# WU-CVGL/CasualHDRSplat

Measured on AMD Instinct MI355X. Metric: train-step images/sec (fwd+bwd raster) @ 1M Gaussians 1080p, higher is better.
Workload: dtype f32; 1 GPU; c3: 1000000 Gaussians, 1920x1080, SH degree 3, HDR radiance + CRF tone-map, 1 pose(s)/view, 1 view(s)/step (one per GPU); num_rendered_R=6777809, R_prime=3025699, pixel_pair_evals_E=559372855, seed=0, binning=sync-free fixed capacity 1.25*R, launch=eager (one enqueue per kernel)

## Files before the change

casualhdrsplat_amd/csrc/api.hip:

```cpp
#include <stdarg.h>
#include <stdio.h>
#include <stdlib.h>
#include <string.h>
#include <time.h>
#include <unistd.h>
#include <atomic>

#include "hs_cloud.h"

namespace hs {

static thread_local char g_err[512] = "";

#ifdef HS_TESTING
int fault_injection() {
    static const int mode = [] {
        const char* e = getenv("HS_FAULT_INJECT");
        return (e && !strcmp(e, "sort_ticket")) ? 1 : (e && !strcmp(e, "stalled_chain")) ? 2 : (e && !strcmp(e, "late_block")) ? 3 : 0;
    }();
    return mode;
}
#endif

static std::atomic<int> g_sort_tickets{0};
// ... 89 lines not shown
    l.offsets = carve(I * 4);
    l.cov3D = carve((int64_t)d.P * 6 * 4);
    l.clamped = carve(I);
    l.scan_spine = carve(((I + 255) / 256 + 1) * 4);
    l.binfo = carve(I * 8);
    sz->geom_bytes = o;
    o = 0;
    l.keys_sorted = carve(2 * align_up(d.capacity * 4, 256));
    l.point_list = l.keys_sorted + align_up(d.capacity * 4, 256);
    l.pairs_tmp = carve(d.capacity * 8);
    l.ranges = carve(vtiles * 8);
    l.sort_tmp = carve(sort_tmp_bytes(I));
    l.depth_ws = carve(depth_ws_words(I) * 4);
    l.depth_pairs = carve(2 * I * 8);
    l.inst_sorted = carve(I * 4);
    l.offs_sorted = carve(I * 4);
    l.pair_sort_tmp = carve(emit_scan_words(I) * 4 + sort_tmp_bytes(d.capacity));
    l.pair_flags = carve(d.capacity);
    l.pair_act = carve(d.capacity);
    l.tile_matrix = carve(count_matrix_words(I, vtiles, d.capacity) * 4);
    l.hier_ws = carve(hier_ws_words(I, gx, gy, d.n_poses, d.capacity) * 4);
    sz->binning_bytes = o;
    o = 0;
    l.final_T = carve(HW * d.n_poses * 4);
    l.n_contrib = carve(HW * d.n_poses * 4);
    l.pose_hdr = carve(HW * 3 * 4 * (d.n_poses + (npf > 1 ? F : 0)));
    l.tile_work = carve(vtiles * 4);
    l.tile_order = carve(vtiles * 4);
    sz->image_bytes = o;
    o = 0;
    l.pair_grads = carve(d.capacity * kPairFloats * 4);
    l.crf_partials = carve(crf_partial_floats(d.crf_K, HW, d.n_poses) * 4);
    l.inst_grads = carve(I * kInstFloats * 4);
    l.pose_partials = carve(pose_partial_floats(d.P, d.n_poses) * 4);
    sz->bwd_bytes = o;
    if (L) *L = l;
    return HS_OK;
}

static int debug_sync(int flags, hipStream_t s, const char* stage) {
    if (!(flags & HS_FLAG_DEBUG)) return HS_OK;
    const hipError_t e = hipStreamSynchronize(s);
    if (e != hipSuccess) {
        set_error("debug: stage `%s` failed: %s", stage, hipGetErrorString(e));
        return HS_EHIP;
    }
    return HS_OK;
}

static int check_common(const hs_dims& d, const float* means3D, const float* shs, const float* colors,
                        const float* scales, const float* rots, const float* cov, const float* view,
                        const float* proj, const float* campos, const float* bg, const char* who) {
    if (!means3D || !view || !proj || !campos || !bg) { set_error("%s: null required pointer", who); return HS_EINVAL; }
    if ((shs == nullptr) == (colors == nullptr)) { set_error("%s: provide exactly one of shs / colors_precomp", who); return HS_EINVAL; }
    const bool sr = scales && rots;
    if (sr == (cov != nullptr) || ((scales == nullptr) != (rots == nullptr))) {
        set_error("%s: provide exactly one of (scales, rotations) / cov3D_precomp", who);
        return HS_EINVAL;
    }
    if (shs) {
        if (d.M > 32) {
            set_error("%s: M=%d SH coefficients per channel; at most 32 are supported", who, d.M);
            return HS_EINVAL;
        }
        if (d.sh_degree < 0 || d.sh_degree > 3 || (d.sh_degree + 1) * (d.sh_degree + 1) > d.M) {
            set_error("%s: sh_degree %d needs %d coefficients, M=%d", who, d.sh_degree, (d.sh_degree + 1) * (d.sh_degree + 1), d.M);
// ... 160 lines not shown
        return HS_EINVAL;
    }
    const int ndens = (a->densify_grad_accum != nullptr) + (a->densify_denom != nullptr) + (a->densify_max_radii != nullptr);
    if (ndens != 0 && ndens != 3) {
        set_error("hs_backward: densification statistics need grad_accum, denom and max_radii together");
        return HS_EINVAL;
    }
    if (a->g_begin != 0 || a->g_end != 0) {
        if (a->g_begin < 0 || a->g_end < a->g_begin || a->g_end > a->dims.P || (a->g_begin & 127) ||
            (a->stages & ~HS_BWD_PROJECT)) {
            set_error("hs_backward: [g_begin, g_end) = [%d, %d) needs 0 <= g_begin <= g_end <= P, g_begin a multiple of 128, "
                      "and stages == HS_BWD_PROJECT", a->g_begin, a->g_end);
            return HS_EINVAL;
        }
    }
    if (a->dims.P == 0) return HS_OK;
    const bool crf_in_tail = HS_TUNE_CRF_IN_RENDER_TAIL && (a->stages & HS_BWD_RENDER) && (a->stages & HS_BWD_CRF) &&
                             !(a->flags & HS_FLAG_DEBUG) && a->crf_K <= 1024;
    if (a->stages & HS_BWD_RENDER) {
        rc = launch_render_bwd(*a, L, s, nullptr, nullptr, crf_in_tail);
        if (rc) return rc;
        if ((rc = debug_sync(a->flags, s, "render backward"))) return rc;
    }
    CrfReduce crf_reduce{nullptr, 0, 0, 0, nullptr, nullptr, 0};
    const bool sums_follow = (a->stages & (HS_BWD_PREPROCESS | HS_BWD_SEGSUM)) != 0 && !(a->flags & HS_FLAG_DEBUG);
    if (a->stages & HS_BWD_CRF) {
        rc = launch_crf_bwd(*a, L, s, sums_follow ? &crf_reduce : nullptr, crf_in_tail);
        if (rc) return rc;
        if ((rc = debug_sync(a->flags, s, "CRF gradient"))) return rc;
    }
    if (a->stages & (HS_BWD_PREPROCESS | HS_BWD_SEGSUM | HS_BWD_PROJECT)) {
        const bool whole = (a->stages & HS_BWD_PREPROCESS) != 0;
        rc = launch_preprocess_bwd(*a, L, s, whole || (a->stages & HS_BWD_SEGSUM), whole || (a->stages & HS_BWD_PROJECT),
                                   crf_reduce.nblocks ? &crf_reduce : nullptr);
        if (rc) return rc;
        if ((rc = debug_sync(a->flags, s, "preprocess backward"))) return rc;
    }
    return HS_OK;
}

int hs_depth_sort(int mode) {
    if (mode >= 0) hs::g_depth_sort.store(mode ? 1 : 0, std::memory_order_relaxed);
    const int v = hs::g_depth_sort.load(std::memory_order_relaxed);
    return v >= 0 ? v : (HS_TUNE_DEPTH_MSD_DEFAULT ? 1 : 0);
}

int hs_sort_tickets(int enable) {
    if (enable >= 0) hs::g_sort_tickets.store(enable ? 1 : 0, std::memory_order_relaxed);
    return hs::g_sort_tickets.load(std::memory_order_relaxed);
}

int hs_mark_visible(int32_t P, const float* means3D, const float* viewmatrix, uint8_t* visible, void* hip_stream) {
    if (P < 0 || (P > 0 && (!means3D || !viewmatrix || !visible))) { set_error("hs_mark_visible: bad argument"); return HS_EINVAL; }
    if (P == 0) return HS_OK;
    return launch_mark_visible(P, means3D, viewmatrix, visible, (hipStream_t)hip_stream);
}

int hs_sh_backward_views(int32_t P, int32_t M, int32_t sh_degree, int32_t V, const float* means3D, const float* camposes,
                         const float* dL_dview_colors, float* dL_dshs, void* hip_stream) {
    if (P < 0 || V < 1 || sh_degree < 0 || sh_degree > 3 || M < (sh_degree + 1) * (sh_degree + 1) || M > 16 ||
        (P > 0 && (!means3D || !camposes || !dL_dview_colors || !dL_dshs))) {
        set_error("hs_sh_backward_views: bad argument");
        return HS_EINVAL;
    }
    if (P == 0) return HS_OK;
    return launch_sh_backward_views(P, M, sh_degree, V, means3D, camposes, dL_dview_colors, dL_dshs, (hipStream_t)hip_stream);
}
// ... 130 lines not shown
```

casualhdrsplat_amd/csrc/hs_common.h:

```cpp
#pragma once
#include <hip/hip_runtime.h>
#include <stdint.h>

#include "../../include/hdrsplat.h"

#if defined(__HIP_DEVICE_COMPILE__) && !defined(__gfx950__)
#error "libhdrsplat is written for gfx950 (MI355X) only: build with --offload-arch=gfx950"
#endif

namespace hs {

void set_error(const char* fmt, ...);

#define HS_HIP_CHECK(expr)                                                                         \
    do {                                                                                           \
        hipError_t e_ = (expr);                                                                    \
        if (e_ != hipSuccess) {                                                                    \
            ::hs::set_error("%s failed: %s (%s:%d)", #expr, hipGetErrorString(e_), __FILE__, __LINE__); \
            return HS_EHIP;                                                                        \
        }                                                                                          \
    } while (0)
#define HS_LAUNCH_CHECK() HS_HIP_CHECK(hipGetLastError())

#ifndef HS_TUNE_CRF_IN_RENDER_TAIL
// ... 18 lines not shown
#endif
constexpr int kDepthSortItems = HS_TUNE_DEPTH_ITEMS, kDepthSortLook = 8;
constexpr int kPairSortItems = 16, kPairSortLook = 8;
constexpr int kU64SortItems = 16;
constexpr int kDepthTile = kDepthSortItems * kDepthBins, kPairTile = kPairSortItems * kSortBlock, kU64Tile = kU64SortItems * kSortBlock;
static_assert(kPairTile == kU64Tile && kDepthTile >= kPairTile, "the scratch of every sort is sized for the smallest tile");
constexpr int kSortTileMin = kPairTile;

static inline int64_t align_up(int64_t v, int64_t a) { return (v + a - 1) / a * a; }
static inline int ceil_div(int64_t a, int64_t b) { return (int)((a + b - 1) / b); }
constexpr int kMaxPoses = 21845;
static inline int frames_of(const hs_dims& d) { return d.n_frames > 1 ? d.n_frames : 1; }

static inline int tile_bits(uint32_t n) {
    int b = 0;
    while (n) { ++b; n >>= 1; }
    return b;
}

int launch_preprocess_fwd(const hs_fwd_args& a, const hs_layout& L, hipStream_t s, uint32_t frame_tag);
int launch_scan(const hs_fwd_args& a, const hs_layout& L, hipStream_t s);
int launch_cov3d(const hs_fwd_args& a, const hs_layout& L, hipStream_t s);
struct SortChoice;
int launch_binning(const hs_fwd_args& a, const hs_layout& L, const SortChoice& sort, hipStream_t s, uint32_t frame_tag);
int launch_empty_frame(hs_counters* clear, uint2* ranges, int64_t ntiles, uint32_t* counters_host, const hs_counters* counters,
                       hipStream_t s);
int launch_render_fwd(const hs_fwd_args& a, const hs_layout& L, hipStream_t s, unsigned long long* stats = nullptr);
int launch_render_bwd(const hs_bwd_args& a, const hs_layout& L, hipStream_t s, unsigned long long* stats = nullptr,
                      unsigned long long* timeline = nullptr, bool crf_in_tail = false);
int render_stats_count();
struct CrfReduce;
int launch_crf_bwd(const hs_bwd_args& a, const hs_layout& L, hipStream_t s, CrfReduce* defer, bool in_render_tail = false);
int launch_preprocess_bwd(const hs_bwd_args& a, const hs_layout& L, hipStream_t s, bool segsum, bool project,
                          const CrfReduce* crf_reduce);
int launch_mark_visible(int P, const float* means3D, const float* view, uint8_t* vis, hipStream_t s);
int launch_spline_poses(int J, int T, int kind, const float* delta, const float* base, const float* times, float* w2c,
                        float* jac, int* seg, hipStream_t s);
int launch_sh_backward_views(int P, int M, int deg, int V, const float* means3D, const float* camposes,
                             const float* view_colors, float* d_shs, hipStream_t s);
int64_t loss_pair_count(int planes, int H, int W);
int launch_loss_fwd(const hs_loss_args& a, hipStream_t s);
int launch_loss_bwd(const hs_loss_args& a, hipStream_t s);
int launch_activate_fwd(const hs_activate_args& a, hipStream_t s);
int launch_activate_bwd(const hs_activate_args& a, hipStream_t s);

constexpr int kGhistCopies = 16;
constexpr int kGhistWords = kGhistCopies * 8 * 256;
constexpr int kTicketWords = 128, kDepthBitsAt = 32, kDepthBitsCopies = 16, kDepthBitsWords = 4 * kDepthBitsCopies;
static_assert(kDepthBitsAt >= 8 && kDepthBitsAt % 2 == 0 && kDepthBitsAt + kDepthBitsWords <= kTicketWords, "depth bits live in the ticket row");
__host__ __device__ inline int64_t sweep_pass_words(int64_t nblk, int bins = 256) { return nblk * bins; }
static inline int64_t sort_scratch_words(int64_t n, int passes, int tile, int bins = 256) {
    return n > 0 ? kGhistWords + kTicketWords + (int64_t)passes * sweep_pass_words((n + tile - 1) / tile, bins) : 0;
}
static inline int64_t depth_scratch_words(int64_t I) { return sort_scratch_words(I, 4, kDepthTile, kDepthBins); }
int64_t sort_tmp_bytes(int64_t n);
constexpr int kMsdBits = 12, kMsdBuckets = 1 << kMsdBits;
#ifndef HS_TUNE_MSD_RANGE
#define HS_TUNE_MSD_RANGE 2048
#endif
constexpr int kMsdRange = HS_TUNE_MSD_RANGE, kMsdCap = 4096;
#ifndef HS_TUNE_MSD_SMALL_RANGE
#define HS_TUNE_MSD_SMALL_RANGE 512
#endif
static inline int depth_msd_range(int64_t I) { return I <= (1 << 18) ? HS_TUNE_MSD_SMALL_RANGE : kMsdRange; }
static inline bool depth_msd_fits(int64_t I) { return I > 0 && I < (2 << 20); }
static inline int depth_msd_tile(int64_t I) { return I <= (1 << 18) ? 1024 : 4096; }
static inline int64_t depth_msd_rows(int64_t I) { return (I + depth_msd_tile(I) - 1) / depth_msd_tile(I); }
// ... 124 lines not shown
}
__device__ __forceinline__ uint32_t wave_or_hi(uint32_t v) {
    v |= dpp_u32<0xB1>(v);
    v |= dpp_u32<0x4E>(v);
    v |= dpp_u32<0x141>(v);
    v |= dpp_u32<0x140>(v);
    v |= dpp_u32<0x142, 0xA>(v);
    v |= dpp_u32<0x143, 0xC>(v);
    return v;
}
__device__ __forceinline__ void depth_bits_accumulate2(uint32_t o_in, uint32_t nz_in, unsigned long long* bits, uint32_t tag,
                                                       uint32_t* s_two ) {
    const uint32_t o = wave_or_hi(o_in), nz = wave_or_hi(nz_in);
    if ((threadIdx.x & 63) == 63) { if (o) atomicOr(&s_two[0], o); if (nz) atomicOr(&s_two[1], nz); }
    __syncthreads();
    if (threadIdx.x < 2 && s_two[threadIdx.x])
        tagged_or(bits + 2 * (blockIdx.x % kDepthBitsCopies) + threadIdx.x, tag, s_two[threadIdx.x]);
}
__device__ __forceinline__ void depth_bits_accumulate(uint32_t key, bool visible, unsigned long long* bits, uint32_t tag,
                                                      uint32_t* s_two ) {
    depth_bits_accumulate2(visible ? key : 0u, visible ? ~key : 0u, bits, tag, s_two);
}
__device__ __forceinline__ float radiance_dact(int act, float col, bool was_clamped) {
    if (act == 1) return col;
    if (act == 2) return -expm1f(-col);
    return was_clamped ? 0.f : 1.f;
}

struct SegsumArgs {
    int64_t I;
    const uint32_t* inst_sorted; const uint32_t* offs_sorted;
    const float4* pair_grads; const uint8_t* pair_flags; float4* inst_grads; const hs_counters* counters;
    const int* radii_inst; const uint8_t* clamped; float* view_colors; const float4* rec; int act;
};
__device__ __forceinline__ void pair_segsum_body(const SegsumArgs& a, int64_t t) {
    const int64_t i = t >> 2;
    const int q = (int)(t & 3);
    const bool valid = i < a.I && !a.counters->overflow;
    const uint32_t beg = valid ? (i == 0 ? 0u : a.offs_sorted[i - 1]) : 0u;
    const uint32_t end = valid ? a.offs_sorted[i] : 0u;
    float r[10] = {0.f, 0.f, 0.f, 0.f, 0.f, 0.f, 0.f, 0.f, 0.f, 0.f};
    for (uint32_t s = beg + q; s < end; s += 8) {
        const bool two = s + 4 < end;
        const bool f0 = a.pair_flags[s] != 0;
        const bool f1 = two && a.pair_flags[s + 4] != 0;
        float4 a0 = make_float4(0.f, 0.f, 0.f, 0.f), a1 = a0, b0 = a0, b1 = a0;
        float2 a2 = make_float2(0.f, 0.f), b2 = a2;
        if (f0) {
            a0 = a.pair_grads[kPairF4 * (int64_t)s + 0];
            a1 = a.pair_grads[kPairF4 * (int64_t)s + 1];
            a2 = reinterpret_cast<const float2*>(a.pair_grads + kPairF4 * (int64_t)s + 2)[0];
        }
        if (f1) {
            b0 = a.pair_grads[kPairF4 * (int64_t)(s + 4) + 0];
            b1 = a.pair_grads[kPairF4 * (int64_t)(s + 4) + 1];
            b2 = reinterpret_cast<const float2*>(a.pair_grads + kPairF4 * (int64_t)(s + 4) + 2)[0];
        }
        r[0] += a0.x; r[1] += a0.y; r[2] += a0.z; r[3] += a0.w;
        r[4] += a1.x; r[5] += a1.y; r[6] += a1.z; r[7] += a1.w;
        r[8] += a2.x; r[9] += a2.y;
        r[0] += b0.x; r[1] += b0.y; r[2] += b0.z; r[3] += b0.w;
        r[4] += b1.x; r[5] += b1.y; r[6] += b1.z; r[7] += b1.w;
        r[8] += b2.x; r[9] += b2.y;
    }
#pragma unroll
    for (int k = 0; k < 10; ++k) {
        r[k] += __shfl_xor(r[k], 1);
        r[k] += __shfl_xor(r[k], 2);
    }
    if (i < a.I && q == 0) {
        const int64_t inst = a.counters->overflow >= 2u ? i : (int64_t)a.inst_sorted[i];
        float4* o = a.inst_grads + kInstF4 * inst;
        o[0] = make_float4(r[0], r[1], r[2], r[3]);
        o[1] = make_float4(r[4], r[5], r[6], r[7]);
        o[2] = make_float4(r[8], r[9], 0.f, 0.f);
        if constexpr (kInstF4 == 4) o[3] = make_float4(0.f, 0.f, 0.f, 0.f);
        if (a.view_colors) {
            const uint8_t cl = a.clamped[inst];
            const bool on = a.radii_inst[inst] > 0;
            float col[3] = {0.f, 0.f, 0.f};
            if (a.act != 0 && on) {
                const float4 rb = a.rec[kRecF4 * inst + 1];
                col[0] = rb.z; col[1] = rb.w; col[2] = reinterpret_cast<const float*>(a.rec + kRecF4 * inst + 2)[0];
            }
            a.view_colors[3 * inst + 0] = on ? radiance_dact(a.act, col[0], cl & 1) * r[6] : 0.f;
            a.view_colors[3 * inst + 1] = on ? radiance_dact(a.act, col[1], cl & 2) * r[7] : 0.f;
            a.view_colors[3 * inst + 2] = on ? radiance_dact(a.act, col[2], cl & 4) * r[8] : 0.f;
        }
    }
}

__device__ __forceinline__ float xform_row(const float* m, int i, float x, float y, float z) {
    return ((m[i] * x + m[4 + i] * y) + m[8 + i] * z) + m[12 + i];
}

}
```

casualhdrsplat_amd/csrc/preprocess.hip:

```cpp
#include "hs_common.h"


namespace hs {

namespace {

__device__ constexpr float SH_C0 = 0.28209479177387814f;
__device__ constexpr float SH_C1 = 0.4886025119029199f;
__device__ constexpr float SH_C2[5] = {1.0925484305920792f, -1.0925484305920792f, 0.31539156525252005f,
                                       -1.0925484305920792f, 0.5462742152960396f};
__device__ constexpr float SH_C3[7] = {-0.5900435899266435f, 2.890611442640554f, -0.4570457994644658f,
                                       0.3731763325901154f,  -0.4570457994644658f, 1.445305721320277f,
                                       -0.5900435899266435f};

struct Ewa {
    float tx, ty, tz;
    bool clamp_x, clamp_y;
    float a0[3], a1[3];
    float fx, fy;
};

__device__ __forceinline__ void quat_to_R(const float* q, float* R) {
    float r = q[0], x = q[1], y = q[2], z = q[3];
    R[0] = 1.f - 2.f * (y * y + z * z); R[1] = 2.f * (x * y - r * z);       R[2] = 2.f * (x * z + r * y);
// ... 342 lines not shown
#pragma unroll
        for (int k = 0; k < 6; ++k) s6[k] = cov_pre[6 * (int64_t)g + k];
    } else {
        float sc[3] = {scales[3 * g], scales[3 * g + 1], scales[3 * g + 2]};
        const float4 q4 = reinterpret_cast<const float4*>(rots)[g];
        float q[4] = {q4.x, q4.y, q4.z, q4.w};
        cov3d_from_scale_rot(sc, mod, q, s6);
    }
#pragma unroll
    for (int k = 0; k < 6; ++k) cov3D[6 * (int64_t)g + k] = s6[k];
}

__global__ void mark_visible_kernel(int P, const float* means, const float* V, uint8_t* vis) {
    int i = blockIdx.x * 256 + threadIdx.x;
    if (i >= P) return;
    vis[i] = xform_row(V, 2, means[3 * i], means[3 * i + 1], means[3 * i + 2]) > 0.2f;
}

__global__ void __launch_bounds__(256) pair_segsum_kernel(SegsumArgs sg, CrfReduce crf_reduce) {
    for (int b = blockIdx.x; b < crf_reduce.nblocks; b += gridDim.x) crf_reduce_block(crf_reduce, b);
    pair_segsum_body(sg, (int64_t)blockIdx.x * 256 + threadIdx.x);
}

struct PreBwd {
    int P, M, W, H, N;
    float tanfovx, tanfovy, mod;
    const float* view; const float* proj; const float* campos;
    const float* means; const float* shs; const float* scales; const float* rots; const float* opac;
    bool has_colors_precomp, has_cov_pre, antialias;
    int act;
    const float4* rec; const int* radii_inst; const uint32_t* tiles; const uint32_t* offsets; const float* cov_pre;
    const uint8_t* clamped;
    const float4* inst_grads;
    float* d_means3D; float* d_means2D; float* d_opac; float* d_shs; float* d_colors; float* d_scales;
    float* d_rots; float* d_cov;
    float* dens_grad; float* dens_denom; int* dens_radii;
    int NF;
    float* pose_partials;
    int blk0;
};

constexpr int kPoseVals = 28;

constexpr int kPreBwdBlock = 128;

__device__ __forceinline__ void stage_rows_in(float* s_rows, const float* src, int rows, int M3, int ld) {
    if ((M3 & 3) == 0 && (reinterpret_cast<uintptr_t>(src) & 15) == 0) {
        const int q = M3 >> 2;
        const float4* src4 = reinterpret_cast<const float4*>(src);
        for (int i = threadIdx.x; i < rows * q; i += kPreBwdBlock) {
            const float4 v = src4[i];
            const int r = i / q;
            float* d = s_rows + r * ld + ((i - r * q) << 2);
            d[0] = v.x; d[1] = v.y; d[2] = v.z; d[3] = v.w;
        }
    } else {
        for (int i = threadIdx.x; i < rows * M3; i += kPreBwdBlock) s_rows[(i / M3) * ld + (i % M3)] = src[i];
    }
}
#ifndef HS_TUNE_PB_UNROLL
#define HS_TUNE_PB_UNROLL 1
#endif
template <int Q>
__device__ __forceinline__ void stage_rows_issue(float4 (&v)[Q > 0 ? Q : 1], const float* src) {
    const float4* src4 = reinterpret_cast<const float4*>(src);
#pragma unroll
    for (int j = 0; j < Q; ++j) v[j] = src4[j * kPreBwdBlock + threadIdx.x];
}
template <int Q>
__device__ __forceinline__ void stage_rows_commit(float* s_rows, const float4 (&v)[Q > 0 ? Q : 1], int ld) {
#pragma unroll
    for (int j = 0; j < Q; ++j) {
        const int i = j * kPreBwdBlock + threadIdx.x;
        const int r = i / Q;
        float* d = s_rows + r * ld + ((i - r * Q) << 2);
        d[0] = v[j].x; d[1] = v[j].y; d[2] = v[j].z; d[3] = v[j].w;
    }
}
__device__ __forceinline__ void stage_rows_out(float* dst, const float* s_rows, int rows, int M3, int ld) {
    if ((M3 & 3) == 0 && (reinterpret_cast<uintptr_t>(dst) & 15) == 0) {
        const int q = M3 >> 2;
        float4* dst4 = reinterpret_cast<float4*>(dst);
        for (int i = threadIdx.x; i < rows * q; i += kPreBwdBlock) {
            const int r = i / q;
            const float* sr = s_rows + r * ld + ((i - r * q) << 2);
            typedef float v4f __attribute__((ext_vector_type(4)));
            __builtin_nontemporal_store(v4f{sr[0], sr[1], sr[2], sr[3]}, reinterpret_cast<v4f*>(dst4) + i);
        }
    } else {
        for (int i = threadIdx.x; i < rows * M3; i += kPreBwdBlock) dst[i] = s_rows[(i / M3) * ld + (i % M3)];
    }
}

#ifndef HS_TUNE_PB_WAVES
#define HS_TUNE_PB_WAVES 0
#endif
#if HS_TUNE_PB_WAVES > 0
#define HS_PB_OCC __attribute__((amdgpu_waves_per_eu(HS_TUNE_PB_WAVES, HS_TUNE_PB_WAVES)))
#else
#define HS_PB_OCC
#endif
template <int DEG, bool POSE, bool SHG>
__global__ void __launch_bounds__(kPreBwdBlock) HS_PB_OCC preprocess_bwd_kernel(PreBwd p) {
    extern __shared__ float s_sh[];
    __shared__ float s_pose[kPreBwdBlock / 64][kPoseVals];
    constexpr int NC = (DEG + 1) * (DEG + 1);
    const int blk = (int)blockIdx.x + p.blk0;
    const int g0 = blk * kPreBwdBlock;
    const int g = g0 + threadIdx.x;
    const int M3 = p.M * 3, ld = M3 + 1;
    const int rows = min(kPreBwdBlock, p.P - g0);
    const bool stage_in = !p.has_colors_precomp && DEG >= 1;
    constexpr int Q = (3 * NC) % 4 == 0 && HS_TUNE_PB_UNROLL ? 3 * NC / 4 : 0;
    float4 staged[Q > 0 ? Q : 1];
    bool fast_stage = false;
    if constexpr (Q > 0) {
        const float* src = p.shs + (int64_t)g0 * M3;
        fast_stage = stage_in && M3 == 3 * NC && rows == kPreBwdBlock && (reinterpret_cast<uintptr_t>(src) & 15) == 0;
        if (fast_stage) stage_rows_issue<Q>(staged, src);
    }
    const bool valid = g < p.P;
    const float x = valid ? p.means[3 * g] : 0.f, y = valid ? p.means[3 * g + 1] : 0.f, z = valid ? p.means[3 * g + 2] : 0.f;
    float s6[6] = {0.f, 0.f, 0.f, 0.f, 0.f, 0.f};
    float4 rot4 = make_float4(0.f, 0.f, 0.f, 0.f);
    float scl[3] = {0.f, 0.f, 0.f};
    if (valid) {
        if (p.cov_pre) {
#pragma unroll
            for (int k = 0; k < 6; ++k) s6[k] = p.cov_pre[6 * (int64_t)g + k];
        } else {
            scl[0] = p.scales[3 * g]; scl[1] = p.scales[3 * g + 1]; scl[2] = p.scales[3 * g + 2];
            rot4 = reinterpret_cast<const float4*>(p.rots)[g];
        }
    }
    const int rad0 = valid ? p.radii_inst[g] : 0;
    float4 pre_q0 = make_float4(0.f, 0.f, 0.f, 0.f), pre_q1 = pre_q0;
    float2 pre_q2 = make_float2(0.f, 0.f);
    uint8_t pre_cl = 0;
    if (rad0 > 0) {
        pre_q0 = p.inst_grads[kInstF4 * (int64_t)g + 0]; pre_q1 = p.inst_grads[kInstF4 * (int64_t)g + 1];
        pre_q2 = reinterpret_cast<const float2*>(p.inst_grads + kInstF4 * (int64_t)g + 2)[0];
        if (!p.has_colors_precomp) pre_cl = p.clamped[g];
    }
    if (stage_in) {
        if (fast_stage) { if constexpr (Q > 0) stage_rows_commit<Q>(s_sh, staged, ld); }
        else stage_rows_in(s_sh, p.shs + (int64_t)g0 * M3, rows, M3, ld);
    }
    if (stage_in) __syncthreads();
    float gm[3] = {0.f, 0.f, 0.f};
    float gcov[6] = {0.f, 0.f, 0.f, 0.f, 0.f, 0.f};
    float gm2d[2] = {0.f, 0.f};
    float gop = 0.f;
    float gcol_pre[3] = {0.f, 0.f, 0.f};

    if (valid && !p.cov_pre) {
        const float q[4] = {rot4.x, rot4.y, rot4.z, rot4.w};
        cov3d_from_scale_rot(scl, p.mod, q, s6);
    }

    int max_radius = 0;
    const bool dens_frames = p.dens_grad != nullptr && p.NF < p.N;
    float fm2d[2] = {0.f, 0.f};
    bool frame_on = false;
    int frame_last = p.NF - 1;
    for (int pose = 0; pose < p.N; ++pose) {
        const int64_t idx = (int64_t)pose * p.P + g;
        const int rad = pose == 0 ? rad0 : (valid ? p.radii_inst[idx] : 0);
        const bool on = rad > 0;
        if (on) max_radius = max(max_radius, rad);
        float pg[POSE ? kPoseVals : 1];
        if constexpr (POSE) {
#pragma unroll
            for (int k = 0; k < kPoseVals; ++k) pg[k] = 0.f;
        }
        if (on) {
        float r[9];
        float r9;
        {
            float4 q0 = pre_q0, q1 = pre_q1;
            float2 q2 = pre_q2;
            if (pose != 0) {
                q0 = p.inst_grads[kInstF4 * idx + 0]; q1 = p.inst_grads[kInstF4 * idx + 1];
                q2 = reinterpret_cast<const float2*>(p.inst_grads + kInstF4 * idx + 2)[0];
            }
            r[0] = q0.x; r[1] = q0.y; r[2] = q0.z; r[3] = q0.w; r[4] = q1.x; r[5] = q1.y; r[6] = q1.z; r[7] = q1.w;
            r[8] = q2.x;
            r9 = q2.y;
        }
        gm2d[0] += r[0]; gm2d[1] += r[1];
        if (dens_frames) { fm2d[0] += r[0]; fm2d[1] += r[1]; frame_on = true; }
        if (!p.antialias) gop += r[5];

        const float* V = p.view + 16 * pose;
        const float* PM = p.proj + 16 * pose;
        const float pvx = xform_row(V, 0, x, y, z), pvy = xform_row(V, 1, x, y, z), pvz = xform_row(V, 2, x, y, z);
        Ewa e;
        ewa_setup(V, p.W, p.H, p.tanfovx, p.tanfovy, pvx, pvy, pvz, e);
        float u0[3], u1[3];
        sym_mul(s6, e.a0, u0);
        sym_mul(s6, e.a1, u1);
        const float a = dot3(e.a0, u0) + 0.3f, b = dot3(e.a1, u0), cc = dot3(e.a1, u1) + 0.3f;
        const float denom = a * cc - b * b;
        const float denom2inv = 1.0f / ((denom * denom) + 0.0000001f);
        const float gA = r[2], gB = r[3], gC = r[4];
        float aa_da = 0.f, aa_db = 0.f, aa_dc = 0.f;
        if (p.antialias) {
            const float det0 = (a - 0.3f) * (cc - 0.3f) - b * b;
            const float q = det0 / denom;
            const float sfac = sqrtf(fmaxf(0.000025f, q));
            gop += r[5] * sfac;
            if (q > 0.000025f) {
                const float k = r[5] * p.opac[g] * 0.5f / sfac / (denom * denom);
                aa_da = k * ((cc - 0.3f) * denom - det0 * cc);
                aa_dc = k * ((a - 0.3f) * denom - det0 * a);
                aa_db = k * (2.f * b * (det0 - denom));
            }
// ... 159 lines not shown
        const float r = q[0], qx = q[1], qy = q[2], qz = q[3];
        if (p.d_scales) { p.d_scales[3 * g] = dsc[0]; p.d_scales[3 * g + 1] = dsc[1]; p.d_scales[3 * g + 2] = dsc[2]; }
        if (p.d_rots) {
            float4 o;
            o.x = 2.f * (-qz * dR[1] + qy * dR[2] + qz * dR[3] - qx * dR[5] - qy * dR[6] + qx * dR[7]);
            o.y = 2.f * (qy * dR[1] + qz * dR[2] + qy * dR[3] - 2.f * qx * dR[4] - r * dR[5] + qz * dR[6] + r * dR[7] - 2.f * qx * dR[8]);
            o.z = 2.f * (-2.f * qy * dR[0] + qx * dR[1] + r * dR[2] + qx * dR[3] + qz * dR[5] - r * dR[6] + qz * dR[7] - 2.f * qy * dR[8]);
            o.w = 2.f * (-2.f * qz * dR[0] - r * dR[1] + qx * dR[2] + r * dR[3] - 2.f * qz * dR[4] + qy * dR[5] + qx * dR[6] + qy * dR[7]);
            reinterpret_cast<float4*>(p.d_rots)[g] = o;
        }
    } else if (valid && p.d_cov) {
#pragma unroll
        for (int k = 0; k < 6; ++k) p.d_cov[6 * (int64_t)g + k] = gcov[k];
    }
    if (valid && p.dens_grad && max_radius > 0) {
        if (!dens_frames) {
            p.dens_grad[g] += sqrtf(gm2d[0] * gm2d[0] + gm2d[1] * gm2d[1]);
            p.dens_denom[g] += 1.f;
        }
        p.dens_radii[g] = max(p.dens_radii[g], max_radius);
    }
    if (valid) {
        if (p.d_means3D) { p.d_means3D[3 * g] = gm[0]; p.d_means3D[3 * g + 1] = gm[1]; p.d_means3D[3 * g + 2] = gm[2]; }
        if (p.d_means2D) { p.d_means2D[3 * g] = gm2d[0]; p.d_means2D[3 * g + 1] = gm2d[1]; p.d_means2D[3 * g + 2] = 0.f; }
        if (p.d_opac) p.d_opac[g] = gop;
        if (p.has_colors_precomp && p.d_colors) {
            p.d_colors[3 * g] = gcol_pre[0]; p.d_colors[3 * g + 1] = gcol_pre[1]; p.d_colors[3 * g + 2] = gcol_pre[2];
        }
    }
    if constexpr (SHG) {
        if (!p.has_colors_precomp && p.d_shs) {
            float* row = s_sh + threadIdx.x * ld;
            for (int k = 0; k < M3; ++k) row[k] = 0.f;
            if (valid) {
                for (int pose = 0; pose < p.N; ++pose) {
                    const int64_t idx = (int64_t)pose * p.P + g;
                    if ((pose == 0 ? rad0 : p.radii_inst[idx]) <= 0) continue;
                    const float4 q1 = pose == 0 ? pre_q1 : p.inst_grads[kInstF4 * idx + 1];
                    const float q2 = pose == 0 ? pre_q2.x : reinterpret_cast<const float*>(p.inst_grads + kInstF4 * idx + 2)[0];
                    const uint8_t cl = pose == 0 ? pre_cl : p.clamped[idx];
                    float col[3] = {0.f, 0.f, 0.f};
                    if (p.act != 0) {
                        const float4 rb = p.rec[kRecF4 * idx + 1];
                        col[0] = rb.z; col[1] = rb.w; col[2] = reinterpret_cast<const float*>(p.rec + kRecF4 * idx + 2)[0];
                    }
                    const float gc[3] = {radiance_dact(p.act, col[0], cl & 1) * q1.z, radiance_dact(p.act, col[1], cl & 2) * q1.w,
                                         radiance_dact(p.act, col[2], cl & 4) * q2};
                    const float* cp = p.campos + 3 * pose;
                    const float dx = x - cp[0], dy = y - cp[1], dz = z - cp[2];
                    const float len = sqrtf((dx * dx + dy * dy) + dz * dz);
                    float bs[NC];
                    sh_basis<DEG>(dx / len, dy / len, dz / len, bs);
#pragma unroll
                    for (int k = 0; k < NC; ++k) {
                        row[3 * k + 0] += bs[k] * gc[0];
                        row[3 * k + 1] += bs[k] * gc[1];
                        row[3 * k + 2] += bs[k] * gc[2];
                    }
                }
            }
            __syncthreads();
            float* dst = p.d_shs + (int64_t)g0 * M3;
            stage_rows_out(dst, s_sh, rows, M3, ld);
        }
    }
}

template <int DEG>
__global__ void __launch_bounds__(kPreBwdBlock) sh_views_kernel(int P, int M, int V, const float* means, const float* campos,
                                                                const float* view_colors, float* d_shs) {
    extern __shared__ float s_sh[];
    constexpr int NC = (DEG + 1) * (DEG + 1);
// ... 93 lines not shown
    p.binfo = (uint2*)(geom + L.binfo);
    p.antialias = (a.flags & HS_FLAG_ANTIALIAS) != 0;
    p.act = (a.flags & HS_FLAG_RADIANCE_EXP) ? 1 : (a.flags & HS_FLAG_RADIANCE_SOFTPLUS) ? 2 : 0;
    p.depth_pairs = nullptr; p.counters = nullptr; p.ranges = nullptr; p.n_vtiles = 0;
    p.sort_zero = nullptr; p.n_sort_zero = 0; p.bits_at = 0; p.frame_tag = 0u;
    p.pair_zero = nullptr; p.n_pair_zero = 0;
    if ((a.stages & HS_STAGE_BIN) && a.binning) {
        char* bin = (char*)a.binning;
        p.depth_pairs = (uint2*)(bin + L.depth_pairs);
        p.counters = (hs_counters*)(geom + L.counters); p.ranges = (uint2*)(bin + L.ranges);
        p.n_vtiles = (int64_t)((d.W + kTile - 1) / kTile) * ((d.H + kTile - 1) / kTile) * d.n_poses;
        p.sort_zero = (uint32_t*)(bin + L.sort_tmp);
        p.n_sort_zero = depth_scratch_words((int64_t)d.P * d.n_poses);
        p.bits_at = kGhistWords + kDepthBitsAt;
        p.frame_tag = frame_tag;
        p.pair_zero = (uint32_t*)(bin + L.pair_sort_tmp);
        p.n_pair_zero = pair_scratch_words((int64_t)d.P * d.n_poses, d.capacity,
                                           sort_passes(tile_bits((uint32_t)p.n_vtiles)));
    }
    if (d.n_poses > 1 && d.P > 0) fill_i32_kernel<<<ceil_div((int64_t)d.P, 1024), 256, 0, s>>>(a.radii, (int64_t)d.P, 0);
    const int grid = (int)(ceil_div(ceil_div((int64_t)d.P, 256), 8) * 8 * d.n_poses);
    const int deg = a.colors_precomp ? 0 : d.sh_degree;
    switch (deg) {
        case 0: preprocess_fwd_kernel<0><<<grid, 256, 0, s>>>(p); break;
        case 1: preprocess_fwd_kernel<1><<<grid, 256, 0, s>>>(p); break;
        case 2: preprocess_fwd_kernel<2><<<grid, 256, 0, s>>>(p); break;
        default: preprocess_fwd_kernel<3><<<grid, 256, 0, s>>>(p); break;
    }
    HS_LAUNCH_CHECK();
    return HS_OK;
}

int launch_preprocess_bwd(const hs_bwd_args& a, const hs_layout& L, hipStream_t s, bool segsum, bool project,
                          const CrfReduce* crf_reduce) {
    const hs_dims& d = a.dims;
    const char* geom = (const char*)a.geom;
    PreBwd p;
    p.P = d.P; p.M = d.M; p.W = d.W; p.H = d.H; p.N = d.n_poses;
    p.tanfovx = a.tanfovx; p.tanfovy = a.tanfovy; p.mod = a.scale_modifier;
    p.view = a.viewmatrices; p.proj = a.projmatrices; p.campos = a.camposes;
    p.means = a.means3D; p.shs = a.shs; p.scales = a.scales; p.rots = a.rotations; p.opac = a.opacities;
    p.antialias = (a.flags & HS_FLAG_ANTIALIAS) != 0;
    p.act = (a.flags & HS_FLAG_RADIANCE_EXP) ? 1 : (a.flags & HS_FLAG_RADIANCE_SOFTPLUS) ? 2 : 0;
    p.has_colors_precomp = a.colors_precomp != nullptr; p.has_cov_pre = a.cov3D_precomp != nullptr;
    p.rec = (const float4*)(geom + L.rec); p.radii_inst = (const int*)(geom + L.radii);
    p.tiles = (const uint32_t*)(geom + L.tiles_touched); p.offsets = (const uint32_t*)(geom + L.offsets);
    p.cov_pre = a.cov3D_precomp; p.clamped = (const uint8_t*)(geom + L.clamped);
    p.inst_grads = (const float4*)((const char*)a.bwd + L.inst_grads);
    const CrfReduce no_reduce{nullptr, 0, 0, 0, nullptr, nullptr, 0};
    if (segsum) {
        const int64_t I = (int64_t)d.P * d.n_poses;
        const char* bin = (const char*)a.binning;
        SegsumArgs sg;
        sg.I = I; sg.inst_sorted = (const uint32_t*)(bin + L.inst_sorted); sg.offs_sorted = (const uint32_t*)(bin + L.offs_sorted);
        sg.pair_grads = (const float4*)((const char*)a.bwd + L.pair_grads); sg.pair_flags = (const uint8_t*)bin + L.pair_flags;
        sg.inst_grads = (float4*)((char*)a.bwd + L.inst_grads); sg.counters = (const hs_counters*)(geom + L.counters);
        sg.radii_inst = p.radii_inst; sg.clamped = p.clamped;
        sg.view_colors = a.colors_precomp ? nullptr : a.dL_dview_colors; sg.rec = p.rec; sg.act = p.act;
        pair_segsum_kernel<<<ceil_div(4 * I, 256), 256, 0, s>>>(sg, crf_reduce ? *crf_reduce : no_reduce);
        HS_LAUNCH_CHECK();
    }
    if (!project) return HS_OK;
    p.d_means3D = a.dL_dmeans3D; p.d_means2D = a.dL_dmeans2D; p.d_opac = a.dL_dopacities; p.d_shs = a.dL_dshs;
    p.d_colors = a.dL_dcolors_precomp; p.d_scales = a.dL_dscales; p.d_rots = a.dL_drotations;
    p.d_cov = a.dL_dcov3D_precomp;
    p.dens_grad = a.densify_grad_accum; p.dens_denom = a.densify_denom; p.dens_radii = a.densify_max_radii;
    p.NF = d.n_poses / frames_of(d);
    const bool shg = p.d_shs != nullptr;
    const bool ranged = a.g_begin != 0 || a.g_end != 0;
    const int g_lo = ranged ? a.g_begin : 0, g_hi = ranged ? a.g_end : d.P;
    const int nblk_all = ceil_div(d.P, kPreBwdBlock);
    const int grid = ceil_div(g_hi - g_lo, kPreBwdBlock);
    p.blk0 = g_lo / kPreBwdBlock;
    const int deg = a.colors_precomp ? 0 : d.sh_degree;
    const size_t lds = (size_t)kPreBwdBlock * (d.M * 3 + 1) * sizeof(float);
    float* pose_partials = a.dL_dviewmatrices ? (float*)((char*)a.bwd + L.pose_partials) : nullptr;
    p.pose_partials = pose_partials;
#define HS_LAUNCH_PRE_BWD(DEG_)                                                                              \
    if (pose_partials && shg) preprocess_bwd_kernel<DEG_, true, true><<<grid, kPreBwdBlock, lds, s>>>(p);       \
    else if (pose_partials) preprocess_bwd_kernel<DEG_, true, false><<<grid, kPreBwdBlock, lds, s>>>(p);        \
    else if (shg) preprocess_bwd_kernel<DEG_, false, true><<<grid, kPreBwdBlock, lds, s>>>(p);                  \
    else preprocess_bwd_kernel<DEG_, false, false><<<grid, kPreBwdBlock, lds, s>>>(p)
    if (grid > 0) switch (deg) {
        case 0: HS_LAUNCH_PRE_BWD(0); break;
        case 1: HS_LAUNCH_PRE_BWD(1); break;
        case 2: HS_LAUNCH_PRE_BWD(2); break;
        default: HS_LAUNCH_PRE_BWD(3); break;
    }
#undef HS_LAUNCH_PRE_BWD
    HS_LAUNCH_CHECK();
    if (pose_partials && g_hi >= d.P) {
// ... 44 lines not shown
```

Measured before the change: 933.1 images/s.

## Skip backward preprocess work for instances without any active pair gradients

The pair segment-sum kernel now records a per-instance touched byte, set when any of its sorted pairs carried a gradient flag, and skips writing inst_grads rows for untouched instances. The projection backward kernel reads this map to build per-block ballot masks. It then skips SH row staging, parameter loads and per-pose gradient math for Gaussians untouched in every pose, and skips inst_grads reads for untouched poses. The aim is less memory traffic and ALU work on Gaussians that are visible but contribute nothing. The cost is an extra byte buffer carved after inst_grads plus ballot and flag-check overhead. It also risks reading a stale map when segsum and project run in separate calls.

```diff
diff --git a/casualhdrsplat_amd/csrc/api.hip b/casualhdrsplat_amd/csrc/api.hip
--- a/casualhdrsplat_amd/csrc/api.hip
+++ b/casualhdrsplat_amd/csrc/api.hip
@@ -145,6 +145,7 @@
     l.pair_grads = carve(d.capacity * kPairFloats * 4);
     l.crf_partials = carve(crf_partial_floats(d.crf_K, HW, d.n_poses) * 4);
     l.inst_grads = carve(I * kInstFloats * 4);
+    carve(I);
     l.pose_partials = carve(pose_partial_floats(d.P, d.n_poses) * 4);
     sz->bwd_bytes = o;
     if (L) *L = l;
@@ -371,7 +372,7 @@
     if (a->stages & (HS_BWD_PREPROCESS | HS_BWD_SEGSUM | HS_BWD_PROJECT)) {
         const bool whole = (a->stages & HS_BWD_PREPROCESS) != 0;
         rc = launch_preprocess_bwd(*a, L, s, whole || (a->stages & HS_BWD_SEGSUM), whole || (a->stages & HS_BWD_PROJECT),
-                                   crf_reduce.nblocks ? &crf_reduce : nullptr);
+                                   crf_reduce.nblocks ? &crf_reduce : nullptr, true);
         if (rc) return rc;
         if ((rc = debug_sync(a->flags, s, "preprocess backward"))) return rc;
     }
diff --git a/casualhdrsplat_amd/csrc/hs_common.h b/casualhdrsplat_amd/csrc/hs_common.h
--- a/casualhdrsplat_amd/csrc/hs_common.h
+++ b/casualhdrsplat_amd/csrc/hs_common.h
@@ -74,7 +74,7 @@
 struct CrfReduce;
 int launch_crf_bwd(const hs_bwd_args& a, const hs_layout& L, hipStream_t s, CrfReduce* defer, bool in_render_tail = false);
 int launch_preprocess_bwd(const hs_bwd_args& a, const hs_layout& L, hipStream_t s, bool segsum, bool project,
-                          const CrfReduce* crf_reduce);
+                          const CrfReduce* crf_reduce, bool touched_map = false);
 int launch_mark_visible(int P, const float* means3D, const float* view, uint8_t* vis, hipStream_t s);
 int launch_spline_poses(int J, int T, int kind, const float* delta, const float* base, const float* times, float* w2c,
                         float* jac, int* seg, hipStream_t s);
@@ -265,7 +265,9 @@
     const uint32_t* inst_sorted; const uint32_t* offs_sorted;
     const float4* pair_grads; const uint8_t* pair_flags; float4* inst_grads; const hs_counters* counters;
     const int* radii_inst; const uint8_t* clamped; float* view_colors; const float4* rec; int act;
+    uint8_t* touched = nullptr;
 };
+static inline int64_t inst_touched_offset(int64_t inst_grads, int64_t I) { return inst_grads + align_up(I * kInstFloats * 4, 256); }
 __device__ __forceinline__ void pair_segsum_body(const SegsumArgs& a, int64_t t) {
     const int64_t i = t >> 2;
     const int q = (int)(t & 3);
@@ -273,10 +275,12 @@
     const uint32_t beg = valid ? (i == 0 ? 0u : a.offs_sorted[i - 1]) : 0u;
     const uint32_t end = valid ? a.offs_sorted[i] : 0u;
     float r[10] = {0.f, 0.f, 0.f, 0.f, 0.f, 0.f, 0.f, 0.f, 0.f, 0.f};
+    bool any = false;
     for (uint32_t s = beg + q; s < end; s += 8) {
         const bool two = s + 4 < end;
         const bool f0 = a.pair_flags[s] != 0;
         const bool f1 = two && a.pair_flags[s + 4] != 0;
+        any |= f0 | f1;
         float4 a0 = make_float4(0.f, 0.f, 0.f, 0.f), a1 = a0, b0 = a0, b1 = a0;
         float2 a2 = make_float2(0.f, 0.f), b2 = a2;
         if (f0) {
@@ -301,13 +305,19 @@
         r[k] += __shfl_xor(r[k], 1);
         r[k] += __shfl_xor(r[k], 2);
     }
+    int hit = any;
+    hit |= __shfl_xor(hit, 1);
+    hit |= __shfl_xor(hit, 2);
     if (i < a.I && q == 0) {
         const int64_t inst = a.counters->overflow >= 2u ? i : (int64_t)a.inst_sorted[i];
-        float4* o = a.inst_grads + kInstF4 * inst;
-        o[0] = make_float4(r[0], r[1], r[2], r[3]);
-        o[1] = make_float4(r[4], r[5], r[6], r[7]);
-        o[2] = make_float4(r[8], r[9], 0.f, 0.f);
-        if constexpr (kInstF4 == 4) o[3] = make_float4(0.f, 0.f, 0.f, 0.f);
+        if (a.touched) a.touched[inst] = hit ? 1 : 0;
+        if (!a.touched || hit) {
+            float4* o = a.inst_grads + kInstF4 * inst;
+            o[0] = make_float4(r[0], r[1], r[2], r[3]);
+            o[1] = make_float4(r[4], r[5], r[6], r[7]);
+            o[2] = make_float4(r[8], r[9], 0.f, 0.f);
+            if constexpr (kInstF4 == 4) o[3] = make_float4(0.f, 0.f, 0.f, 0.f);
+        }
         if (a.view_colors) {
             const uint8_t cl = a.clamped[inst];
             const bool on = a.radii_inst[inst] > 0;
diff --git a/casualhdrsplat_amd/csrc/preprocess.hip b/casualhdrsplat_amd/csrc/preprocess.hip
--- a/casualhdrsplat_amd/csrc/preprocess.hip
+++ b/casualhdrsplat_amd/csrc/preprocess.hip
@@ -398,6 +398,7 @@
     const float4* rec; const int* radii_inst; const uint32_t* tiles; const uint32_t* offsets; const float* cov_pre;
     const uint8_t* clamped;
     const float4* inst_grads;
+    const uint8_t* touched = nullptr;
     float* d_means3D; float* d_means2D; float* d_opac; float* d_shs; float* d_colors; float* d_scales;
     float* d_rots; float* d_cov;
     float* dens_grad; float* dens_denom; int* dens_radii;
@@ -410,18 +411,27 @@
 
 constexpr int kPreBwdBlock = 128;
 
-__device__ __forceinline__ void stage_rows_in(float* s_rows, const float* src, int rows, int M3, int ld) {
+static_assert(kPreBwdBlock == 128, "the rows of one block are two 64-bit words of flags");
+__device__ __forceinline__ bool row_wanted(uint64_t lo, uint64_t hi, int r) {
+    const uint64_t w = r < 64 ? lo : hi;
+    return (w >> (r & 63)) & 1u;
+}
+__device__ __forceinline__ void stage_rows_in(float* s_rows, const float* src, int rows, int M3, int ld, uint64_t want_lo, uint64_t want_hi) {
     if ((M3 & 3) == 0 && (reinterpret_cast<uintptr_t>(src) & 15) == 0) {
         const int q = M3 >> 2;
         const float4* src4 = reinterpret_cast<const float4*>(src);
         for (int i = threadIdx.x; i < rows * q; i += kPreBwdBlock) {
+            const int r = i / q;
+            if (!row_wanted(want_lo, want_hi, r)) continue;
             const float4 v = src4[i];
-            const int r = i / q;
             float* d = s_rows + r * ld + ((i - r * q) << 2);
             d[0] = v.x; d[1] = v.y; d[2] = v.z; d[3] = v.w;
         }
     } else {
-        for (int i = threadIdx.x; i < rows * M3; i += kPreBwdBlock) s_rows[(i / M3) * ld + (i % M3)] = src[i];
+        for (int i = threadIdx.x; i < rows * M3; i += kPreBwdBlock) {
+            const int r = i / M3;
+            if (row_wanted(want_lo, want_hi, r)) s_rows[r * ld + (i - r * M3)] = src[i];
+        }
     }
 }
 #ifndef HS_TUNE_PB_UNROLL
@@ -432,6 +442,16 @@
     const float4* src4 = reinterpret_cast<const float4*>(src);
 #pragma unroll
     for (int j = 0; j < Q; ++j) v[j] = src4[j * kPreBwdBlock + threadIdx.x];
+}
+template <int Q>
+__device__ __forceinline__ void stage_rows_issue(float4 (&v)[Q > 0 ? Q : 1], const float* src, uint64_t want_lo, uint64_t want_hi) {
+    const float4* src4 = reinterpret_cast<const float4*>(src);
+#pragma unroll
+    for (int j = 0; j < Q; ++j) {
+        const int i = j * kPreBwdBlock + threadIdx.x;
+        v[j] = make_float4(0.f, 0.f, 0.f, 0.f);
+        if (row_wanted(want_lo, want_hi, i / Q)) v[j] = src4[i];
+    }
 }
 template <int Q>
 __device__ __forceinline__ void stage_rows_commit(float* s_rows, const float4 (&v)[Q > 0 ? Q : 1], int ld) {
@@ -477,20 +497,49 @@
     const int M3 = p.M * 3, ld = M3 + 1;
     const int rows = min(kPreBwdBlock, p.P - g0);
     const bool stage_in = !p.has_colors_precomp && DEG >= 1;
+    uint64_t want_lo = ~0ull, want_hi = ~0ull;
+    uint32_t own_bits = ~0u;
+    if (p.touched) {
+        const int ga = g0 + (int)(threadIdx.x & 63), gb = ga + 64;
+        uint32_t a_any = 0, b_any = 0;
+        own_bits = 0u;
+        for (int p0 = 0; p0 < p.N; p0 += 4) {
+            uint32_t ta[4], tb[4];
+#pragma unroll
+            for (int k = 0; k < 4; ++k) {
+                const bool in = p0 + k < p.N;
+                const uint8_t* m = p.touched + (int64_t)(in ? p0 + k : 0) * p.P;
+                ta[k] = in && ga < p.P ? m[ga] : 0u;
+                tb[k] = in && gb < p.P ? m[gb] : 0u;
+            }
+#pragma unroll
+            for (int k = 0; k < 4; ++k) {
+                a_any |= ta[k]; b_any |= tb[k];
+                if ((threadIdx.x < 64 ? ta[k] : tb[k]) != 0 && p0 + k < 32) own_bits |= 1u << (p0 + k);
+            }
+        }
+        want_lo = __ballot(a_any != 0); want_hi = __ballot(b_any != 0);
+    }
+    const bool own0 = own_bits & 1u;
+    const bool live = row_wanted(want_lo, want_hi, (int)threadIdx.x);
     constexpr int Q = (3 * NC) % 4 == 0 && HS_TUNE_PB_UNROLL ? 3 * NC / 4 : 0;
     float4 staged[Q > 0 ? Q : 1];
     bool fast_stage = false;
     if constexpr (Q > 0) {
         const float* src = p.shs + (int64_t)g0 * M3;
         fast_stage = stage_in && M3 == 3 * NC && rows == kPreBwdBlock && (reinterpret_cast<uintptr_t>(src) & 15) == 0;
-        if (fast_stage) stage_rows_issue<Q>(staged, src);
+        if (fast_stage) {
+            if ((want_lo & want_hi) == ~0ull) stage_rows_issue<Q>(staged, src);
+            else stage_rows_issue<Q>(staged, src, want_lo, want_hi);
+        }
     }
     const bool valid = g < p.P;
-    const float x = valid ? p.means[3 * g] : 0.f, y = valid ? p.means[3 * g + 1] : 0.f, z = valid ? p.means[3 * g + 2] : 0.f;
+    const bool work = valid && live;
+    const float x = work ? p.means[3 * g] : 0.f, y = work ? p.means[3 * g + 1] : 0.f, z = work ? p.means[3 * g + 2] : 0.f;
     float s6[6] = {0.f, 0.f, 0.f, 0.f, 0.f, 0.f};
     float4 rot4 = make_float4(0.f, 0.f, 0.f, 0.f);
     float scl[3] = {0.f, 0.f, 0.f};
-    if (valid) {
+    if (work) {
         if (p.cov_pre) {
 #pragma unroll
             for (int k = 0; k < 6; ++k) s6[k] = p.cov_pre[6 * (int64_t)g + k];
@@ -503,14 +552,16 @@
     float4 pre_q0 = make_float4(0.f, 0.f, 0.f, 0.f), pre_q1 = pre_q0;
     float2 pre_q2 = make_float2(0.f, 0.f);
     uint8_t pre_cl = 0;
-    if (rad0 > 0) {
-        pre_q0 = p.inst_grads[kInstF4 * (int64_t)g + 0]; pre_q1 = p.inst_grads[kInstF4 * (int64_t)g + 1];
-        pre_q2 = reinterpret_cast<const float2*>(p.inst_grads + kInstF4 * (int64_t)g + 2)[0];
+    if (rad0 > 0 && live) {
+        if (own0) {
+            pre_q0 = p.inst_grads[kInstF4 * (int64_t)g + 0]; pre_q1 = p.inst_grads[kInstF4 * (int64_t)g + 1];
+            pre_q2 = reinterpret_cast<const float2*>(p.inst_grads + kInstF4 * (int64_t)g + 2)[0];
+        }
         if (!p.has_colors_precomp) pre_cl = p.clamped[g];
     }
     if (stage_in) {
         if (fast_stage) { if constexpr (Q > 0) stage_rows_commit<Q>(s_sh, staged, ld); }
-        else stage_rows_in(s_sh, p.shs + (int64_t)g0 * M3, rows, M3, ld);
+        else stage_rows_in(s_sh, p.shs + (int64_t)g0 * M3, rows, M3, ld, want_lo, want_hi);
     }
     if (stage_in) __syncthreads();
     float gm[3] = {0.f, 0.f, 0.f};
@@ -533,21 +584,24 @@
         const int64_t idx = (int64_t)pose * p.P + g;
         const int rad = pose == 0 ? rad0 : (valid ? p.radii_inst[idx] : 0);
         const bool on = rad > 0;
-        if (on) max_radius = max(max_radius, rad);
+        if (on) { max_radius = max(max_radius, rad); if (dens_frames) frame_on = true; }
         float pg[POSE ? kPoseVals : 1];
         if constexpr (POSE) {
 #pragma unroll
             for (int k = 0; k < kPoseVals; ++k) pg[k] = 0.f;
         }
-        if (on) {
+        if (on && live) {
         float r[9];
         float r9;
         {
             float4 q0 = pre_q0, q1 = pre_q1;
             float2 q2 = pre_q2;
             if (pose != 0) {
-                q0 = p.inst_grads[kInstF4 * idx + 0]; q1 = p.inst_grads[kInstF4 * idx + 1];
-                q2 = reinterpret_cast<const float2*>(p.inst_grads + kInstF4 * idx + 2)[0];
+                q0 = make_float4(0.f, 0.f, 0.f, 0.f); q1 = q0; q2 = make_float2(0.f, 0.f);
+                if (pose < 32 ? (own_bits >> pose) & 1u : !p.touched || p.touched[idx]) {
+                    q0 = p.inst_grads[kInstF4 * idx + 0]; q1 = p.inst_grads[kInstF4 * idx + 1];
+                    q2 = reinterpret_cast<const float2*>(p.inst_grads + kInstF4 * idx + 2)[0];
+                }
             }
             r[0] = q0.x; r[1] = q0.y; r[2] = q0.z; r[3] = q0.w; r[4] = q1.x; r[5] = q1.y; r[6] = q1.z; r[7] = q1.w;
             r[8] = q2.x;
@@ -773,12 +827,19 @@
         if (!p.has_colors_precomp && p.d_shs) {
             float* row = s_sh + threadIdx.x * ld;
             for (int k = 0; k < M3; ++k) row[k] = 0.f;
-            if (valid) {
+            if (work) {
                 for (int pose = 0; pose < p.N; ++pose) {
                     const int64_t idx = (int64_t)pose * p.P + g;
                     if ((pose == 0 ? rad0 : p.radii_inst[idx]) <= 0) continue;
-                    const float4 q1 = pose == 0 ? pre_q1 : p.inst_grads[kInstF4 * idx + 1];
-                    const float q2 = pose == 0 ? pre_q2.x : reinterpret_cast<const float*>(p.inst_grads + kInstF4 * idx + 2)[0];
+                    float4 q1 = pre_q1;
+                    float q2 = pre_q2.x;
+                    if (pose != 0) {
+                        q1 = make_float4(0.f, 0.f, 0.f, 0.f); q2 = 0.f;
+                        if (pose < 32 ? (own_bits >> pose) & 1u : !p.touched || p.touched[idx]) {
+                            q1 = p.inst_grads[kInstF4 * idx + 1];
+                            q2 = reinterpret_cast<const float*>(p.inst_grads + kInstF4 * idx + 2)[0];
+                        }
+                    }
                     const uint8_t cl = pose == 0 ? pre_cl : p.clamped[idx];
                     float col[3] = {0.f, 0.f, 0.f};
                     if (p.act != 0) {
@@ -938,7 +999,7 @@
 }
 
 int launch_preprocess_bwd(const hs_bwd_args& a, const hs_layout& L, hipStream_t s, bool segsum, bool project,
-                          const CrfReduce* crf_reduce) {
+                          const CrfReduce* crf_reduce, bool touched_map) {
     const hs_dims& d = a.dims;
     const char* geom = (const char*)a.geom;
     PreBwd p;
@@ -953,6 +1014,8 @@
     p.tiles = (const uint32_t*)(geom + L.tiles_touched); p.offsets = (const uint32_t*)(geom + L.offsets);
     p.cov_pre = a.cov3D_precomp; p.clamped = (const uint8_t*)(geom + L.clamped);
     p.inst_grads = (const float4*)((const char*)a.bwd + L.inst_grads);
+    uint8_t* touched = touched_map ? (uint8_t*)a.bwd + inst_touched_offset(L.inst_grads, (int64_t)d.P * d.n_poses) : nullptr;
+    p.touched = touched;
     const CrfReduce no_reduce{nullptr, 0, 0, 0, nullptr, nullptr, 0};
     if (segsum) {
         const int64_t I = (int64_t)d.P * d.n_poses;
@@ -963,6 +1026,7 @@
         sg.inst_grads = (float4*)((char*)a.bwd + L.inst_grads); sg.counters = (const hs_counters*)(geom + L.counters);
         sg.radii_inst = p.radii_inst; sg.clamped = p.clamped;
         sg.view_colors = a.colors_precomp ? nullptr : a.dL_dview_colors; sg.rec = p.rec; sg.act = p.act;
+        sg.touched = touched;
         pair_segsum_kernel<<<ceil_div(4 * I, 256), 256, 0, s>>>(sg, crf_reduce ? *crf_reduce : no_reduce);
         HS_LAUNCH_CHECK();
     }
```

Measured after the change: 979.4 images/s (median of 3 runs). +5.0%, better.
